# myshell-ai/OpenVoice

Hardware: AMD Instinct MI355X
Metric: real_time_factor (higher is better)
Workload: dtype f32; 1 GPU; ToneColorConverter.convert path, 32 x 10 s @ 22.05 kHz per GPU (T=861 frames), fp32, calibrated random weights; batch_per_gpu=32, global_batch=32, parallelism=dp1 (utterance sharding, RCCL broadcast of src/tgt se)

## Files before the change

include/openvoice_amd.h:

```cpp
#ifndef OPENVOICE_AMD_H
#define OPENVOICE_AMD_H

#include <stddef.h>
#include <stdint.h>

#ifdef __cplusplus
extern "C" {
#endif

typedef void* ov_stream_t;

enum {
  OV_OK = 0,
  OV_E_BADARG = -1,
  OV_E_UNSUPPORTED = -2,
  OV_E_ALIGN = -3,
  OV_E_LAUNCH = -4
};

enum {
  OV_EPI_LINEAR = 0,
  OV_EPI_GATE = 1,
  OV_EPI_RESSKIP = 2,
  OV_EPI_COUPLE = 3,
// ... 85 lines not shown
  const float* w_rs;
  const float* b_rs;
  const float* mask;
  int64_t bstride;
  int64_t cond_bstride;
  int64_t mask_bstride;
  int32_t B, H, T;
  int32_t ld;
  int32_t K;
  int32_t first;
  int32_t last;
  int32_t width;
  int32_t ntile;
  int32_t row_split;
  unsigned long long* dbg;
  float* acts;
} ov_wn_layer_params;
int ov_wn_layer_f32(const ov_wn_layer_params* p, ov_stream_t stream);
int ov_wn_layer_supported(int H, int K);
size_t ov_wn_pack_size(int rows, int cin, int K);
int ov_wn_pack_f32(const float* w, int rows, int cin, int K, float* dst);
int ov_wn_layer_tile(int B, int T, int width);

int ov_frame_hops_f32(const float* wave, float* hops, int B, int N, int hop, int pad, int U, int ld,
                      ov_stream_t stream);

int ov_frame_hops_windows_f32(const float* wave, int64_t n_samples, const int64_t* first_frame, int W, int hop, int pad,
                              int U, int ld, float* hops, ov_stream_t stream);
int ov_frame_hops_multi_f32(const float* pool, int64_t pool_len, const int64_t* records, int W, int hop, int pad, int U,
                            int ld, float* hops, ov_stream_t stream);
int ov_stitch_window_cores_f32(const float* o_hat, const int64_t* windows, int W, int Tw, int spf, float* out,
                               int64_t out_len, int64_t out_frame0, ov_stream_t stream);
int ov_carry_rows_f32(const int64_t* records, int n_records, const float* src_base, int64_t src_elems, float* dst_base,
                      int64_t dst_elems, ov_stream_t stream);
int ov_rows_f32_to_cl_bf16(const float* src, int64_t src_bs, int src_ld, uint16_t* dst, int B, int C, int L,
                           ov_stream_t stream);
int ov_cl_bf16_to_rows_f32(const uint16_t* src, float* dst, int64_t dst_bs, int dst_ld, int B, int C, int L,
                           ov_stream_t stream);

int ov_vad_frame_energy_f32(const float* pool, int64_t pool_len, const int64_t* records, int R, int H, int ldT,
                            float* energy, ov_stream_t stream);
int ov_vad_segments_i32(const float* energy, const int64_t* records, int R, int H, int ldT, float floor_lin,
                        float range_lin, int min_silence_frames, int min_speech_frames, int pad_frames, int32_t* mask,
                        int64_t* offsets, int64_t* n_active, ov_stream_t stream);
int ov_vad_compact_f32(const float* pool, int64_t pool_len, const int64_t* records, int R, int H, int ldT,
                       const int32_t* mask, const int64_t* offsets, const int64_t* out_bases, float* out,
// ... 189 lines not shown
```

openvoice_amd/_lib.py:

```python
import ctypes
import os

_HERE = os.path.dirname(os.path.abspath(__file__))
LIB_PATH = os.environ.get("OPENVOICE_AMD_LIB") or os.path.join(_HERE, "libopenvoice_amd.so")

OV_OK = 0
MIN_VERSION = 212
OV_ERRORS = {-1: "OV_E_BADARG", -2: "OV_E_UNSUPPORTED", -3: "OV_E_ALIGN", -4: "OV_E_LAUNCH"}

EPI_LINEAR, EPI_GATE, EPI_RESSKIP, EPI_COUPLE, EPI_POSTERIOR, EPI_CONVT, EPI_MAGNITUDE = range(7)
F_MASK_V = 1
F_OUT2_INIT = 2
F_CONVT_GROUPED = 4
F_NO_XCD_MAP = 8

_fp = ctypes.c_void_p
_i = ctypes.c_int
_i64 = ctypes.c_int64
LN_PRE_RELU, LN_POST_GELU = 1, 2


class ConvParams(ctypes.Structure):
    _fields_ = [
        ("x", _fp), ("w", _fp), ("bias", _fp), ("bias_b", _fp), ("out", _fp), ("res", _fp),
# ... 65 lines not shown
class WnLayerParams(ctypes.Structure):
    _fields_ = [("x", _fp), ("out", _fp), ("skip", _fp), ("w_in", _fp), ("b_in", _fp), ("cond", _fp), ("w_rs", _fp),
                ("b_rs", _fp), ("mask", _fp),
                ("bstride", ctypes.c_int64), ("cond_bstride", ctypes.c_int64), ("mask_bstride", ctypes.c_int64),
                ("B", ctypes.c_int32), ("H", ctypes.c_int32), ("T", ctypes.c_int32), ("ld", ctypes.c_int32),
                ("K", ctypes.c_int32), ("first", ctypes.c_int32), ("last", ctypes.c_int32), ("width", ctypes.c_int32),
                ("ntile", ctypes.c_int32), ("row_split", ctypes.c_int32), ("dbg", _fp), ("acts", _fp)]


SIGNATURES = {
    "ov_version": (ctypes.c_int, []),
    "ov_build_experiment": (ctypes.c_int, []),
    "ov_conv1d_pack_size": (ctypes.c_size_t, [ctypes.c_int, ctypes.c_int, ctypes.c_int]),
    "ov_conv1d_pack_rows": (ctypes.c_int, [ctypes.c_int]),
    "ov_conv1d_pack_f32": (ctypes.c_int, [_fp, ctypes.c_int, ctypes.c_int, ctypes.c_int, _fp]),
    "ov_conv1d_f32": (ctypes.c_int, [ctypes.POINTER(ConvParams), _fp]),
    "ov_resblock_pair_f32": (ctypes.c_int, [ctypes.POINTER(RespairParams), _fp]),
    "ov_resblock_pair_supported": (ctypes.c_int, [_i, _i, _i]),
    "ov_wn_layer_f32": (ctypes.c_int, [ctypes.POINTER(WnLayerParams), _fp]),
    "ov_wn_layer_supported": (ctypes.c_int, [_i, _i]),
    "ov_wn_pack_size": (ctypes.c_size_t, [_i, _i, _i]),
    "ov_wn_pack_f32": (ctypes.c_int, [_fp, _i, _i, _i, _fp]),
    "ov_wn_layer_tile": (ctypes.c_int, [_i, _i, _i]),
    "ov_conv_post_tanh_f32": (ctypes.c_int, [_fp, _fp, _fp, ctypes.c_int, ctypes.c_int, ctypes.c_int,
                                             ctypes.c_int, ctypes.c_float, _fp]),
    "ov_conv_post_tanh_limited_f32": (ctypes.c_int, [_fp, _fp, _fp, ctypes.c_int, ctypes.c_int, ctypes.c_int,
                                                     ctypes.c_int, ctypes.c_float, _fp, ctypes.c_int, _fp]),
    "ov_frame_limits_i32": (ctypes.c_int, [_fp, _fp, _i, _i, _i, _fp]),
    "ov_linear_f32": (ctypes.c_int, [_fp, _fp, _fp, _fp, ctypes.c_int, ctypes.c_int, ctypes.c_int, _fp]),
    "ov_sequence_mask_f32": (ctypes.c_int, [_fp, _fp, ctypes.c_int, ctypes.c_int, ctypes.c_int, _fp]),
    "ov_unpad_rows_f32": (ctypes.c_int, [_fp, _fp, ctypes.c_int, ctypes.c_int, ctypes.c_int, _fp]),
    "ov_polyphase_fir_f32": (ctypes.c_int, [_fp, _fp, _fp, ctypes.c_int64, ctypes.c_int64, _i, _i, _i, _fp]),
    "ov_polyphase_fir_rows_f32": (ctypes.c_int, [_fp, _i, _fp, _i64, _fp, _i64, _fp, _i64, _i64, _fp]),
    "ov_layernorm_freq_f32": (ctypes.c_int, [_fp, _fp, _fp, _fp, ctypes.c_int, ctypes.c_int, ctypes.c_int,
                                             ctypes.c_float, _fp]),
    "ov_conv2d_s2_relu_f32": (ctypes.c_int, [_fp, _fp, _fp, _fp, ctypes.c_int, ctypes.c_int, ctypes.c_int,
                                             ctypes.c_int, ctypes.c_int, _fp]),
    "ov_gru_f32": (ctypes.c_int, [_fp, _fp, _fp, _fp, ctypes.c_int, ctypes.c_int, ctypes.c_int, _fp]),
    "ov_conv1d_bf16_pack_size": (ctypes.c_size_t, [_i, _i, _i]),
    "ov_conv1d_bf16_pack": (ctypes.c_int, [_fp, _i, _i, _i, _fp]),
    "ov_conv1d_bf16_pack16": (ctypes.c_int, [_fp, _i, _i, _i, _fp]),
    "ov_conv1d_bf16cl": (ctypes.c_int, [ctypes.POINTER(ConvBf16Params), _fp]),
    "ov_resblock_pair_bf16cl": (ctypes.c_int, [ctypes.POINTER(RespairBf16Params), _fp]),
    "ov_resblock_pair_bf16_supported": (ctypes.c_int, [_i, _i, _i]),
    "ov_resblock_pair2_bf16cl": (ctypes.c_int, [ctypes.POINTER(Respair2Bf16Params), _fp]),
    "ov_resblock_pair2_bf16_supported": (ctypes.c_int, [_i, _i, _i]),
# ... 68 lines not shown
        _lib = lib
    return _lib


def torch_op(name, *args):
    try:
        return getattr(torch_ops(), name)(*args)
    except RuntimeError as exc:
        if isinstance(exc, OvError):
            raise
        raise OvError(str(exc).split("\n")[0]) from None


def check(code, what):
    if code != OV_OK:
        raise OvError(f"{what} failed: {OV_ERRORS.get(code, code)}")


SHIM_PATH = os.path.join(_HERE, "libopenvoice_amd_torch.so")
_ops = None
VALUE_FUNCS = {"ov_version", "ov_build_experiment", "ov_conv1d_pack_size", "ov_conv1d_pack_rows", "ov_wn_pack_size",
               "ov_conv1d_bf16_pack_size", "ov_resblock_pair_supported", "ov_wn_layer_supported", "ov_wn_layer_tile",
               "ov_resblock_pair_bf16_supported", "ov_resblock_pair2_bf16_supported", "ov_conv1d_split3_pack_size",
               "ov_conv1d_split3_supported", "ov_conv1d_wino_supported", "ov_conv1d_wino_chunk", "ov_conv1d_wino_pack_size"}


def binding():
    b = os.environ.get("OPENVOICE_AMD_BINDING", "ctypes" if os.environ.get("OPENVOICE_AMD_LIB") else "torch")
    if b not in ("torch", "ctypes"):
        raise OvError(f"OPENVOICE_AMD_BINDING={b!r}: expected 'torch' or 'ctypes'")
    return b


def use_torch_binding():
    return binding() == "torch"


def torch_ops():
    global _ops
    if _ops is None:
        import torch
        for path in (LIB_PATH, SHIM_PATH):
            if not os.path.exists(path):
                raise OvError(f"{path} not found: build the HIP extension first (python -c 'import __graft_entry__ "
                              f"as g; g.build()'); there is no CPU fallback (OPENVOICE_AMD_BINDING=ctypes needs only "
                              f"libopenvoice_amd.so)")
        torch.ops.load_library(SHIM_PATH)
# ... 49 lines not shown
```

openvoice_amd/csrc/torch_shim.cpp:

```cpp
#include <ATen/ATen.h>
#include <ATen/hip/impl/HIPGuardImplMasqueradingAsCUDA.h>
#include <c10/hip/HIPStream.h>
#include <torch/library.h>

#include <string>
#include <type_traits>

#include "openvoice_amd.h"

namespace {

const char* ov_strerror(int rc) {
  switch (rc) {
    case OV_E_BADARG: return "OV_E_BADARG";
    case OV_E_UNSUPPORTED: return "OV_E_UNSUPPORTED";
    case OV_E_ALIGN: return "OV_E_ALIGN";
    case OV_E_LAUNCH: return "OV_E_LAUNCH";
    default: return "unknown error";
  }
}

using OptTensor = c10::optional<at::Tensor>;

struct Ctx {
// ... 180 lines not shown
  DeviceScope scope(c);
  finish(ov_conv1d_f32(&p, c.stream()), "ov_conv1d_f32");
}

void resblock_pair_f32(const OptTensor& x, const OptTensor& w1, const OptTensor& b1, const OptTensor& w2,
                       const OptTensor& b2, const OptTensor& out, const OptTensor& add, const OptTensor& dbg,
                       const OptTensor& col_limit, at::IntArrayRef ip, at::ArrayRef<double> fp) {
  TORCH_CHECK(ip.size() == 11 && fp.size() == 2, "openvoice_amd::resblock_pair_f32: 11 integer and 2 float parameters");
  Ctx c{"resblock_pair_f32", false};
  ov_respair_params p{};
  p.x = sptr<float>(x, c, 0); p.w1 = sptr<float>(w1, c, 1); p.b1 = sptr<float>(b1, c, 2);
  p.w2 = sptr<float>(w2, c, 3); p.b2 = sptr<float>(b2, c, 4); p.out = sptr<float>(out, c, 5);
  p.add = sptr<float>(add, c, 6);
  p.dbg = sptr<unsigned long long>(dbg, c, 7);
  p.col_limit = sptr<int32_t>(col_limit, c, 8);
  p.B = (int32_t)ip[0]; p.C = (int32_t)ip[1]; p.L = (int32_t)ip[2]; p.ld = (int32_t)ip[3]; p.K = (int32_t)ip[4];
  p.dil = (int32_t)ip[5]; p.nwg = (int32_t)ip[6];
  p.x_bstride = ip[7]; p.out_bstride = ip[8]; p.add_bstride = ip[9]; p.col_limit_scale = (int32_t)ip[10];
  p.slope = (float)fp[0]; p.scale = (float)fp[1];
  DeviceScope scope(c);
  finish(ov_resblock_pair_f32(&p, c.stream()), "ov_resblock_pair_f32");
}

void wn_layer_f32(const OptTensor& x, const OptTensor& out, const OptTensor& skip, const OptTensor& w_in,
                  const OptTensor& b_in, const OptTensor& cond, const OptTensor& w_rs, const OptTensor& b_rs,
                  const OptTensor& mask, const OptTensor& dbg, const OptTensor& acts, at::IntArrayRef ip) {
  TORCH_CHECK(ip.size() == 13, "openvoice_amd::wn_layer_f32: 13 integer parameters");
  Ctx c{"wn_layer_f32", false};
  ov_wn_layer_params p{};
  p.x = sptr<float>(x, c, 0); p.out = sptr<float>(out, c, 1); p.skip = sptr<float>(skip, c, 2);
  p.w_in = sptr<float>(w_in, c, 3); p.b_in = sptr<float>(b_in, c, 4); p.cond = sptr<float>(cond, c, 5, ip[11]);
  p.w_rs = sptr<float>(w_rs, c, 6); p.b_rs = sptr<float>(b_rs, c, 7); p.mask = sptr<float>(mask, c, 8);
  p.dbg = sptr<unsigned long long>(dbg, c, 9);
  p.acts = sptr<float>(acts, c, 10);
  p.B = (int32_t)ip[0]; p.H = (int32_t)ip[1]; p.T = (int32_t)ip[2]; p.ld = (int32_t)ip[3]; p.K = (int32_t)ip[4];
  p.first = (int32_t)ip[5]; p.last = (int32_t)ip[6]; p.width = (int32_t)ip[7];
  p.bstride = ip[8]; p.cond_bstride = ip[9]; p.mask_bstride = ip[10]; p.row_split = (int32_t)ip[12];
  DeviceScope scope(c);
  finish(ov_wn_layer_f32(&p, c.stream()), "ov_wn_layer_f32");
}

void conv1d_bf16cl(const OptTensor& x, const OptTensor& w, const OptTensor& bias, const OptTensor& out,
                   const OptTensor& res, const OptTensor& add, const OptTensor& dbg, at::IntArrayRef ip,
                   at::ArrayRef<double> fp) {
  TORCH_CHECK(ip.size() == 9 && fp.size() == 3, "openvoice_amd::conv1d_bf16cl: 9 integer and 3 float parameters");
  Ctx c{"conv1d_bf16cl", false};
  ov_conv1d_bf16_params p{};
  p.x = sptr<uint16_t>(x, c, 0); p.w = sptr<uint16_t>(w, c, 1); p.bias = sptr<float>(bias, c, 2);
  p.out = sptr<uint16_t>(out, c, 3); p.res = sptr<uint16_t>(res, c, 4); p.add = sptr<uint16_t>(add, c, 5);
  p.dbg = sptr<unsigned long long>(dbg, c, 6);
  p.B = (int32_t)ip[0]; p.L = (int32_t)ip[1]; p.Cin = (int32_t)ip[2]; p.Cout = (int32_t)ip[3]; p.K = (int32_t)ip[4];
  p.dil = (int32_t)ip[5]; p.phase_s = (int32_t)ip[6]; p.bias_bstride = (int32_t)ip[7]; p.layout = (int32_t)ip[8];
  p.in_slope = (float)fp[0]; p.scale = (float)fp[1]; p.out_slope = (float)fp[2];
  DeviceScope scope(c);
  finish(ov_conv1d_bf16cl(&p, c.stream()), "ov_conv1d_bf16cl");
}

void resblock_pair_bf16cl(const OptTensor& x, const OptTensor& w1, const OptTensor& b1, const OptTensor& w2,
                          const OptTensor& b2, const OptTensor& out, const OptTensor& add, const OptTensor& dbg,
                          at::IntArrayRef ip, at::ArrayRef<double> fp) {
  TORCH_CHECK(ip.size() == 6 && fp.size() == 2, "openvoice_amd::resblock_pair_bf16cl: 6 integer and 2 float parameters");
  Ctx c{"resblock_pair_bf16cl", false};
// ... 50 lines not shown
  Ctx c{"conv1d_wino_f32", false};
  ov_conv1d_wino_params p{};
  p.x = sptr<float>(x, c, 0); p.w = sptr<float>(w, c, 1); p.bias = sptr<float>(bias, c, 2);
  p.out = sptr<float>(out, c, 3); p.res = sptr<float>(res, c, 4); p.add = sptr<float>(add, c, 5);
  p.dbg = sptr<unsigned long long>(dbg, c, 6);
  p.col_limit = sptr<int32_t>(col_limit, c, 7); p.col_limit_scale = (int32_t)ip[14];
  p.B = (int32_t)ip[0]; p.Cin = (int32_t)ip[1]; p.Cout = (int32_t)ip[2]; p.L = (int32_t)ip[3];
  p.x_ld = (int32_t)ip[4]; p.out_ld = (int32_t)ip[5]; p.K = (int32_t)ip[6]; p.dil = (int32_t)ip[7]; p.nwg = (int32_t)ip[8];
  p.x_bstride = ip[9]; p.out_bstride = ip[10]; p.res_bstride = ip[11]; p.add_bstride = ip[12]; p.frags = (int32_t)ip[13];
  p.in_slope = (float)fp[0]; p.scale = (float)fp[1]; p.out_slope = (float)fp[2];
  DeviceScope scope(c);
  finish(ov_conv1d_wino_f32(&p, c.stream()), "ov_conv1d_wino_f32");
}

}

TORCH_LIBRARY(openvoice_amd, m) {
  m.def("conv1d_f32(Tensor? x, Tensor? w, Tensor? bias, Tensor(a!)? out, Tensor? res, Tensor? add, Tensor(b!)? out2, "
        "Tensor? mask, Tensor? bias_b, Tensor? col_limit, int[] ip, float[] fp) -> ()", &conv1d_f32);
  m.def("resblock_pair_f32(Tensor? x, Tensor? w1, Tensor? b1, Tensor? w2, Tensor? b2, Tensor(a!)? out, Tensor? add, "
        "Tensor(b!)? dbg, Tensor? col_limit, int[] ip, float[] fp) -> ()", &resblock_pair_f32);
  m.def("wn_layer_f32(Tensor? x, Tensor(a!)? out, Tensor(b!)? skip, Tensor? w_in, Tensor? b_in, Tensor? cond, Tensor? w_rs, "
        "Tensor? b_rs, Tensor? mask, Tensor(c!)? dbg, Tensor(d!)? acts, int[] ip) -> ()", &wn_layer_f32);
  m.def("conv1d_bf16cl(Tensor? x, Tensor? w, Tensor? bias, Tensor(a!)? out, Tensor? res, Tensor? add, Tensor(b!)? dbg, "
        "int[] ip, float[] fp) -> ()", &conv1d_bf16cl);
  m.def("resblock_pair_bf16cl(Tensor? x, Tensor? w1, Tensor? b1, Tensor? w2, Tensor? b2, Tensor(a!)? out, Tensor? add, "
        "Tensor(b!)? dbg, int[] ip, float[] fp) -> ()", &resblock_pair_bf16cl);
  m.def("resblock_pair2_bf16cl(Tensor? x, Tensor? w1, Tensor? b1, Tensor? w2, Tensor? b2, Tensor(a!)? out, Tensor? add, "
        "Tensor(b!)? dbg, int[] ip, float[] fp) -> ()", &resblock_pair2_bf16cl);
  m.def("conv1d_split3(Tensor? x, Tensor? w, Tensor? bias, Tensor(a!)? out, Tensor? res, Tensor(b!)? dbg, "
        "Tensor? col_limit, int[] ip, float[] fp) -> ()", &conv1d_split3);
  m.def("conv1d_wino_f32(Tensor? x, Tensor? w, Tensor? bias, Tensor(a!)? out, Tensor? res, Tensor? add, Tensor(b!)? dbg, "
        "Tensor? col_limit, int[] ip, float[] fp) -> ()",
        &conv1d_wino_f32);
  bind_device<&ov_frame_hops_f32>(m, "frame_hops_f32");
  bind_device<&ov_frame_hops_windows_f32>(m, "frame_hops_windows_f32");
  bind_device<&ov_frame_hops_multi_f32>(m, "frame_hops_multi_f32");
  bind_device<&ov_carry_rows_f32>(m, "carry_rows_f32");
  bind_device<&ov_rows_f32_to_cl_bf16>(m, "rows_f32_to_cl_bf16");
  bind_device<&ov_cl_bf16_to_rows_f32>(m, "cl_bf16_to_rows_f32");
  bind_device<&ov_vad_frame_energy_f32>(m, "vad_frame_energy_f32");
  bind_device<&ov_vad_segments_i32>(m, "vad_segments_i32");
  bind_device<&ov_vad_compact_f32>(m, "vad_compact_f32");
  bind_device<&ov_stitch_window_cores_f32>(m, "stitch_window_cores_f32");
  bind_device<&ov_conv_post_tanh_f32>(m, "conv_post_tanh_f32");
  bind_device<&ov_conv_post_tanh_limited_f32>(m, "conv_post_tanh_limited_f32");
  bind_device<&ov_frame_limits_i32>(m, "frame_limits_i32");
  bind_device<&ov_linear_f32>(m, "linear_f32");
  bind_device<&ov_sequence_mask_f32>(m, "sequence_mask_f32");
  bind_device<&ov_unpad_rows_f32>(m, "unpad_rows_f32");
  bind_device<&ov_polyphase_fir_f32>(m, "polyphase_fir_f32");
  bind_device<&ov_polyphase_fir_rows_f32>(m, "polyphase_fir_rows_f32");
  bind_device<&ov_layernorm_freq_f32>(m, "layernorm_freq_f32");
  bind_device<&ov_conv2d_s2_relu_f32>(m, "conv2d_s2_relu_f32");
  bind_device<&ov_gru_f32>(m, "gru_f32");
  bind_device<&ov_embed_f32>(m, "embed_f32");
  bind_device<&ov_layernorm_ch_f32>(m, "layernorm_ch_f32");
  bind_device<&ov_rel_attention_f32>(m, "rel_attention_f32");
  bind_device<&ov_dwconv1d_f32>(m, "dwconv1d_f32");
  bind_device<&ov_expand1_f32>(m, "expand1_f32");
  bind_device<&ov_add_bias_mask_f32>(m, "add_bias_mask_f32");
  bind_device<&ov_rq_spline_inverse_f32>(m, "rq_spline_inverse_f32");
  bind_device<&ov_duration_f32>(m, "duration_f32");
  bind_device<&ov_expand_prior_f32>(m, "expand_prior_f32");
  bind_device<&ov_conv_post_tanh_bf16>(m, "conv_post_tanh_bf16");
  bind_device<&ov_split3_from_f32>(m, "split3_from_f32");
  bind_device<&ov_split3_to_f32>(m, "split3_to_f32");
  bind_host<&ov_conv1d_pack_f32>(m, "conv1d_pack_f32");
  bind_host<&ov_wn_pack_f32>(m, "wn_pack_f32");
  bind_host<&ov_conv1d_bf16_pack>(m, "conv1d_bf16_pack");
  bind_host<&ov_conv1d_bf16_pack16>(m, "conv1d_bf16_pack16");
  bind_host<&ov_conv1d_split3_pack>(m, "conv1d_split3_pack");
  bind_value<&ov_conv1d_split3_pack_size>(m, "conv1d_split3_pack_size");
  bind_value<&ov_conv1d_split3_supported>(m, "conv1d_split3_supported");
  bind_host<&ov_conv1d_wino_pack_f32>(m, "conv1d_wino_pack_f32");
  bind_value<&ov_conv1d_wino_pack_size>(m, "conv1d_wino_pack_size");
  bind_value<&ov_conv1d_wino_supported>(m, "conv1d_wino_supported");
  bind_value<&ov_conv1d_wino_chunk>(m, "conv1d_wino_chunk");
  bind_value<&ov_conv1d_pack_size>(m, "conv1d_pack_size");
  bind_value<&ov_conv1d_pack_rows>(m, "conv1d_pack_rows");
  bind_value<&ov_wn_pack_size>(m, "wn_pack_size");
  bind_value<&ov_conv1d_bf16_pack_size>(m, "conv1d_bf16_pack_size");
  bind_value<&ov_resblock_pair_supported>(m, "resblock_pair_supported");
  bind_value<&ov_wn_layer_supported>(m, "wn_layer_supported");
  bind_value<&ov_wn_layer_tile>(m, "wn_layer_tile");
  bind_value<&ov_resblock_pair_bf16_supported>(m, "resblock_pair_bf16_supported");
  bind_value<&ov_resblock_pair2_bf16_supported>(m, "resblock_pair2_bf16_supported");
  bind_value<&ov_version>(m, "version");
  bind_value<&ov_build_experiment>(m, "build_experiment");
}
```

openvoice_amd/engine.py:

```python
import ctypes
import os

import torch

from . import _lib
from ._lib import (ConvParams, EPI_CONVT, EPI_COUPLE, EPI_GATE, EPI_LINEAR, EPI_POSTERIOR, EPI_RESSKIP,
                   F_CONVT_GROUPED, F_MASK_V, F_OUT2_INIT)
from .params import ENC_Q_LAYERS, FLOW_LAYERS, N_FLOWS, REF_ENC_FILTERS, REF_ENC_GRU, effective_weight

GENERATOR_MARGIN = 16
LIMIT_MAX_BATCH = 256
LRELU_SLOPE = 0.1
FINAL_LRELU_SLOPE = 0.01


SUPPORTED_RESBLOCK_KERNELS = (3, 7, 11)
SUPPORTED_RESBLOCK_DILATIONS = (1, 3, 5)


def validate_config(cfg):
    def bad(field, value, why):
        raise _lib.OvError(f"config field {field!r} = {value!r} is not supported by the MI355X kernels: {why}")

    rb = str(cfg.get("resblock", "1"))
# ... 270 lines not shown
    return max(GENERATOR_MARGIN, generator_margin_frames(cfg), generator_margin_frames(cfg, chain_reach=chain_reach))


def wn_fused_row_order(hidden):
    assert hidden % 8 == 0
    idx = []
    for q in range(hidden // 8):
        for j in range(4):
            a, b = 8 * q + j, 8 * q + j + 4
            idx += [a, b, hidden + a, hidden + b]
    return torch.tensor(idx, dtype=torch.long)


def wn_pack(w_dense, device):
    w_dense = w_dense.detach().to(torch.float32).cpu().contiguous()
    rows, cin, k = w_dense.shape
    n = _lib.call("ov_wn_pack_size", rows, cin, k)
    assert n > 0, (rows, cin, k)
    packed = torch.empty(n, dtype=torch.float32)
    _lib.call("ov_wn_pack_f32", w_dense, rows, cin, k, packed)
    return packed.to(device)


def launch_wn_layer(layer, x, out, skip, mask, B, T, ld, cond=None, cond_off=0, cond_bs=0, first=False, last=False,
                    width=0, mask_bs=0, dbg=None, acts=None, row_split=0):
    if _lib.use_torch_binding():
        H = layer["hidden"]
        _lib.torch_op("wn_layer_f32", x, out, skip, layer["w_in"], layer["b_in"], cond, layer["w_rs"], layer["b_rs"],
                      mask, dbg, acts, [B, H, T, ld, layer["K"], int(first), int(last), width, H * ld, cond_bs, mask_bs,
                                        cond_off, row_split])
        return
    p = _lib.WnLayerParams()
    p.x, p.out, p.skip = _ptr(x), _ptr(out), _ptr(skip)
    p.w_in, p.b_in, p.w_rs, p.b_rs = _ptr(layer["w_in"]), _ptr(layer["b_in"]), _ptr(layer["w_rs"]), _ptr(layer["b_rs"])
    p.cond = _ptr(cond, cond_off) if cond is not None else None
    p.mask = _ptr(mask)
    H = layer["hidden"]
    p.bstride, p.cond_bstride, p.mask_bstride = H * ld, cond_bs, mask_bs
    p.B, p.H, p.T, p.ld, p.K = B, H, T, ld, layer["K"]
    p.first, p.last, p.width, p.row_split = int(first), int(last), width, row_split
    p.dbg = ctypes.c_void_p(dbg.data_ptr()) if dbg is not None else None
    p.acts = _ptr(acts) if acts is not None else None
    stream = ctypes.c_void_p(torch.cuda.current_stream(x.device).cuda_stream)
    _lib.check(_lib.load().ov_wn_layer_f32(ctypes.byref(p), stream), "ov_wn_layer_f32")


class _WaveNet:

    def __init__(self, sd, prefix, n_layers, hidden, device):
        order = gate_row_order(hidden)
        self.hidden, self.n_layers = hidden, n_layers
        self.in_layers, self.rs_layers, self.fused_layers = [], [], []
        K = sd[f"{prefix}.in_layers.0.weight_v"].shape[2] if f"{prefix}.in_layers.0.weight_v" in sd else \
            sd[f"{prefix}.in_layers.0.weight"].shape[2]
        self.fused = bool(_lib.call("ov_wn_layer_supported", hidden, K))
        forder = wn_fused_row_order(hidden) if self.fused else None
        for i in range(n_layers):
            w_in = effective_weight(sd, f"{prefix}.in_layers.{i}")
            b_in = sd[f"{prefix}.in_layers.{i}.bias"].float()
            self.in_layers.append(PackedConv(w_in[order], b_in[order], device, K=w_in.shape[2], cout=hidden))
            w_rs = effective_weight(sd, f"{prefix}.res_skip_layers.{i}")
            b_rs = sd[f"{prefix}.res_skip_layers.{i}.bias"].float()
            self.rs_layers.append(PackedConv(w_rs, b_rs, device, K=1))
            if self.fused:
                if w_rs.shape[0] == hidden:
                    w_rs = torch.cat([torch.zeros_like(w_rs), w_rs])
                    b_rs = torch.cat([torch.zeros_like(b_rs), b_rs])
                self.fused_layers.append(dict(hidden=hidden, K=w_in.shape[2], w_in=wn_pack(w_in[forder], device),
                                              b_in=b_in[forder].contiguous().to(device), w_rs=wn_pack(w_rs, device),
                                              b_rs=b_rs.contiguous().to(device)))
        wc = effective_weight(sd, prefix + ".cond_layer")[:, :, 0]
        bc = sd[prefix + ".cond_layer.bias"].float()
        full = torch.cat([order + 2 * hidden * i for i in range(n_layers)])
        self.cond_w = wc[full].contiguous().to(device)
        self.cond_b = bc[full].contiguous().to(device)
        if self.fused:
            full = torch.cat([forder + 2 * hidden * i for i in range(n_layers)])
            self.cond_w_fused = wc[full].contiguous().to(device)
            self.cond_b_fused = bc[full].contiguous().to(device)


class ConverterEngine:

    def __init__(self, state_dict, model_cfg, spec_channels, device, zero_g=False):
        self.device = torch.device(device)
        if self.device.type != "cuda":
            raise _lib.OvError("ConverterEngine needs a ROCm device ('cuda:N'); there is no CPU path")
        sd = {k: v.detach().float().cpu() for k, v in state_dict.items()}
        cfg = dict(model_cfg.items()) if hasattr(model_cfg, "items") else dict(model_cfg)
        validate_config(cfg)
        self.cfg = cfg
# ... 195 lines not shown
    def _zeros_like_cached(self, t):
        key = tuple(t.shape)
        z = self._zeros.get(key)
        if z is None:
            z = self._zeros[key] = torch.zeros_like(t)
        return z

    def _side_streams(self, n):
        while len(self._streams) < n:
            self._streams.append(torch.cuda.Stream(self.device))
        return self._streams[:n]

    def _chain_scratch(self, ws, n):
        extra = ws.setdefault("dec_extra", [])
        while len(extra) < n:
            extra.append(torch.empty_like(ws["dec"][0]))
        return extra

    def _wavenet(self, wn, ws, B, T, cond, mask):
        H, Tp = wn.hidden, ws["Tp"]
        cbs = 0 if cond.shape[0] == 1 else cond.shape[1]
        if self.fuse_wn and wn.fused:
            src, dst = ws["h"], ws["h2"]
            for i in range(wn.n_layers):
                layer = wn.fused_layers[i]
                args = dict(cond=cond, cond_off=2 * H * i, cond_bs=cbs, first=i == 0, last=i == wn.n_layers - 1,
                            mask_bs=Tp, acts=ws["acts"], row_split=self.wn_row_split)
                if self.profile is None:
                    launch_wn_layer(layer, src, dst, ws["skip"], mask, B, T, Tp, **args)
                else:
                    e0, e1 = torch.cuda.Event(enable_timing=True), torch.cuda.Event(enable_timing=True)
                    e0.record()
                    launch_wn_layer(layer, src, dst, ws["skip"], mask, B, T, Tp, **args)
                    e1.record()
                    rs_rows = H if args["last"] else 2 * H
                    self.profile.append(("wn_layer", 2.0 * (2 * H * H * layer["K"] + rs_rows * H) * T * B, e0, e1))
                src, dst = dst, src
            return
        for i in range(wn.n_layers):
            self._conv(wn.in_layers[i], ws["h"], 0, H * Tp, ws["acts"], 0, H * Tp, B, T, epi=EPI_GATE,
                       bias_b=cond, bias_b_off=2 * H * i, bias_b_bs=cbs, rows=2 * H, x_ld=Tp, out_ld=Tp, tag="wn_in")
            last = i == wn.n_layers - 1
            self._conv(wn.rs_layers[i], ws["acts"], 0, H * Tp, ws["h"], 0, H * Tp, B, T, epi=EPI_RESSKIP,
                       flags=F_OUT2_INIT if i == 0 else 0, out2=ws["skip"], out2_bs=H * Tp, mask=mask, mask_bs=Tp,
                       split=0 if last else H, x_ld=Tp, out_ld=Tp, tag="wn_rs")

    def _flow(self, src, buf, ws, B, T, conds, mask, reverse):
        C, half, H, Tp = self.inter, self.half, self.hidden, ws["Tp"]
        order = range(N_FLOWS - 1, -1, -1) if reverse else range(N_FLOWS)
        for n, f in enumerate(order):
# ... 516 lines not shown
```

Before: 3060 x real-time (audio s / wall s).

## Add Winograd-based fused WaveNet layer kernel for K=5, H=192

Adds a fused WaveNet layer kernel whose dilated K=5 input convolution uses a Winograd F(4,3)-style transform split into two 3-tap groups, running on MFMA f32 16x16x4 with double-buffered LDS transforms, then the gate and res/skip 1x1 conv in the same kernel. Weights are pre-transformed on the host into a new packed layout, and a policy based on tile count per occupancy round chooses it when enabled. The aim is to cut multiply count for the input conv. The trade-offs are extra transform arithmetic, reduced fp32 accuracy from the transform constants, and a fixed 128-wide tile that can hurt wave quantization.

```diff
diff --git a/include/openvoice_amd.h b/include/openvoice_amd.h
--- a/include/openvoice_amd.h
+++ b/include/openvoice_amd.h
@@ -131,6 +131,11 @@
 int ov_wn_pack_f32(const float* w, int rows, int cin, int K, float* dst);
 int ov_wn_layer_tile(int B, int T, int width);
 
+int ov_wn_layer_wino_f32(const ov_wn_layer_params* p, ov_stream_t stream);
+int ov_wn_layer_wino_tile(void);
+size_t ov_wn_wino_pack_size(int rows, int cin, int K);
+int ov_wn_wino_pack_f32(const float* w, int rows, int cin, int K, float* dst);
+
 int ov_frame_hops_f32(const float* wave, float* hops, int B, int N, int hop, int pad, int U, int ld,
                       ov_stream_t stream);
 
diff --git a/openvoice_amd/_lib.py b/openvoice_amd/_lib.py
--- a/openvoice_amd/_lib.py
+++ b/openvoice_amd/_lib.py
@@ -111,6 +111,10 @@
     "ov_wn_pack_size": (ctypes.c_size_t, [_i, _i, _i]),
     "ov_wn_pack_f32": (ctypes.c_int, [_fp, _i, _i, _i, _fp]),
     "ov_wn_layer_tile": (ctypes.c_int, [_i, _i, _i]),
+    "ov_wn_layer_wino_f32": (ctypes.c_int, [ctypes.POINTER(WnLayerParams), _fp]),
+    "ov_wn_layer_wino_tile": (ctypes.c_int, []),
+    "ov_wn_wino_pack_size": (ctypes.c_size_t, [_i, _i, _i]),
+    "ov_wn_wino_pack_f32": (ctypes.c_int, [_fp, _i, _i, _i, _fp]),
     "ov_conv_post_tanh_f32": (ctypes.c_int, [_fp, _fp, _fp, ctypes.c_int, ctypes.c_int, ctypes.c_int,
                                              ctypes.c_int, ctypes.c_float, _fp]),
     "ov_conv_post_tanh_limited_f32": (ctypes.c_int, [_fp, _fp, _fp, ctypes.c_int, ctypes.c_int, ctypes.c_int,
@@ -225,7 +229,8 @@
 VALUE_FUNCS = {"ov_version", "ov_build_experiment", "ov_conv1d_pack_size", "ov_conv1d_pack_rows", "ov_wn_pack_size",
                "ov_conv1d_bf16_pack_size", "ov_resblock_pair_supported", "ov_wn_layer_supported", "ov_wn_layer_tile",
                "ov_resblock_pair_bf16_supported", "ov_resblock_pair2_bf16_supported", "ov_conv1d_split3_pack_size",
-               "ov_conv1d_split3_supported", "ov_conv1d_wino_supported", "ov_conv1d_wino_chunk", "ov_conv1d_wino_pack_size"}
+               "ov_conv1d_split3_supported", "ov_conv1d_wino_supported", "ov_conv1d_wino_chunk", "ov_conv1d_wino_pack_size",
+               "ov_wn_layer_wino_tile", "ov_wn_wino_pack_size"}
 
 
 def binding():
diff --git a/openvoice_amd/csrc/torch_shim.cpp b/openvoice_amd/csrc/torch_shim.cpp
--- a/openvoice_amd/csrc/torch_shim.cpp
+++ b/openvoice_amd/csrc/torch_shim.cpp
@@ -226,11 +226,13 @@
   finish(ov_resblock_pair_f32(&p, c.stream()), "ov_resblock_pair_f32");
 }
 
-void wn_layer_f32(const OptTensor& x, const OptTensor& out, const OptTensor& skip, const OptTensor& w_in,
-                  const OptTensor& b_in, const OptTensor& cond, const OptTensor& w_rs, const OptTensor& b_rs,
-                  const OptTensor& mask, const OptTensor& dbg, const OptTensor& acts, at::IntArrayRef ip) {
-  TORCH_CHECK(ip.size() == 13, "openvoice_amd::wn_layer_f32: 13 integer parameters");
-  Ctx c{"wn_layer_f32", false};
+template <int (*FN)(const ov_wn_layer_params*, ov_stream_t)>
+void wn_layer_any(const char* op, const char* entry, const OptTensor& x, const OptTensor& out, const OptTensor& skip,
+                  const OptTensor& w_in, const OptTensor& b_in, const OptTensor& cond, const OptTensor& w_rs,
+                  const OptTensor& b_rs, const OptTensor& mask, const OptTensor& dbg, const OptTensor& acts,
+                  at::IntArrayRef ip) {
+  TORCH_CHECK(ip.size() == 13, "openvoice_amd::", op, ": 13 integer parameters");
+  Ctx c{op, false};
   ov_wn_layer_params p{};
   p.x = sptr<float>(x, c, 0); p.out = sptr<float>(out, c, 1); p.skip = sptr<float>(skip, c, 2);
   p.w_in = sptr<float>(w_in, c, 3); p.b_in = sptr<float>(b_in, c, 4); p.cond = sptr<float>(cond, c, 5, ip[11]);
@@ -241,7 +243,18 @@
   p.first = (int32_t)ip[5]; p.last = (int32_t)ip[6]; p.width = (int32_t)ip[7];
   p.bstride = ip[8]; p.cond_bstride = ip[9]; p.mask_bstride = ip[10]; p.row_split = (int32_t)ip[12];
   DeviceScope scope(c);
-  finish(ov_wn_layer_f32(&p, c.stream()), "ov_wn_layer_f32");
+  finish(FN(&p, c.stream()), entry);
+}
+void wn_layer_f32(const OptTensor& x, const OptTensor& out, const OptTensor& skip, const OptTensor& w_in,
+                  const OptTensor& b_in, const OptTensor& cond, const OptTensor& w_rs, const OptTensor& b_rs,
+                  const OptTensor& mask, const OptTensor& dbg, const OptTensor& acts, at::IntArrayRef ip) {
+  wn_layer_any<&ov_wn_layer_f32>("wn_layer_f32", "ov_wn_layer_f32", x, out, skip, w_in, b_in, cond, w_rs, b_rs, mask, dbg, acts, ip);
+}
+void wn_layer_wino_f32(const OptTensor& x, const OptTensor& out, const OptTensor& skip, const OptTensor& w_in,
+                       const OptTensor& b_in, const OptTensor& cond, const OptTensor& w_rs, const OptTensor& b_rs,
+                       const OptTensor& mask, const OptTensor& dbg, const OptTensor& acts, at::IntArrayRef ip) {
+  wn_layer_any<&ov_wn_layer_wino_f32>("wn_layer_wino_f32", "ov_wn_layer_wino_f32", x, out, skip, w_in, b_in, cond, w_rs, b_rs, mask, dbg,
+                                      acts, ip);
 }
 
 void conv1d_bf16cl(const OptTensor& x, const OptTensor& w, const OptTensor& bias, const OptTensor& out,
@@ -338,6 +351,8 @@
         "Tensor(b!)? dbg, Tensor? col_limit, int[] ip, float[] fp) -> ()", &resblock_pair_f32);
   m.def("wn_layer_f32(Tensor? x, Tensor(a!)? out, Tensor(b!)? skip, Tensor? w_in, Tensor? b_in, Tensor? cond, Tensor? w_rs, "
         "Tensor? b_rs, Tensor? mask, Tensor(c!)? dbg, Tensor(d!)? acts, int[] ip) -> ()", &wn_layer_f32);
+  m.def("wn_layer_wino_f32(Tensor? x, Tensor(a!)? out, Tensor(b!)? skip, Tensor? w_in, Tensor? b_in, Tensor? cond, Tensor? w_rs, "
+        "Tensor? b_rs, Tensor? mask, Tensor(c!)? dbg, Tensor(d!)? acts, int[] ip) -> ()", &wn_layer_wino_f32);
   m.def("conv1d_bf16cl(Tensor? x, Tensor? w, Tensor? bias, Tensor(a!)? out, Tensor? res, Tensor? add, Tensor(b!)? dbg, "
         "int[] ip, float[] fp) -> ()", &conv1d_bf16cl);
   m.def("resblock_pair_bf16cl(Tensor? x, Tensor? w1, Tensor? b1, Tensor? w2, Tensor? b2, Tensor(a!)? out, Tensor? add, "
@@ -384,6 +399,9 @@
   bind_device<&ov_split3_to_f32>(m, "split3_to_f32");
   bind_host<&ov_conv1d_pack_f32>(m, "conv1d_pack_f32");
   bind_host<&ov_wn_pack_f32>(m, "wn_pack_f32");
+  bind_host<&ov_wn_wino_pack_f32>(m, "wn_wino_pack_f32");
+  bind_value<&ov_wn_wino_pack_size>(m, "wn_wino_pack_size");
+  bind_value<&ov_wn_layer_wino_tile>(m, "wn_layer_wino_tile");
   bind_host<&ov_conv1d_bf16_pack>(m, "conv1d_bf16_pack");
   bind_host<&ov_conv1d_bf16_pack16>(m, "conv1d_bf16_pack16");
   bind_host<&ov_conv1d_split3_pack>(m, "conv1d_split3_pack");
diff --git a/openvoice_amd/csrc/wn_layer_wino.hip b/openvoice_amd/csrc/wn_layer_wino.hip
--- /dev/null
+++ b/openvoice_amd/csrc/wn_layer_wino.hip
@@ -0,0 +1,354 @@
+#include <hip/hip_runtime.h>
+
+#include "conv1d_wino.h"
+#include "openvoice_amd.h"
+
+namespace ovkwn {
+
+using ovk::f32x2;
+using ovk::f32x4;
+using ovkw::lds_barrier;
+using ovkw::wino_products;
+using ovkw::wino_zero_product;
+
+constexpr int K = 5, H = 192;
+static_assert(ovkw::wino_lead(K) == 0 && ovkw::wino_trail(K) == 1 && wino_products(K) == 11, "(w0 w1 w2)(w3 w4 0)");
+constexpr int NWAVE = 8;
+constexpr int RB = 2 * H / (16 * NWAVE);
+constexpr int NF = 2;
+constexpr int NT = 16 * NF;
+constexpr int W = 4 * NT;
+constexpr int NB = W / 16;
+constexpr int CI = 16;
+constexpr int NCH = H / CI;
+constexpr int NSLOT = wino_products(K);
+constexpr int SLOT = CI * NT;
+constexpr int VBUF = NSLOT * SLOT;
+constexpr int NU = H / 4;
+constexpr int XS = 144;
+constexpr int NR2 = H / 16;
+static_assert(NWAVE * 64 == CI * NT, "one (channel, tile) per lane and chunk");
+
+__device__ __forceinline__ float gate(float t, float s) {
+  const float a = __builtin_amdgcn_exp2f(fabsf(t) * -2.8853900817779268f);
+  const float e = __builtin_amdgcn_exp2f(s * -1.4426950408889634f);
+  const float r = __builtin_amdgcn_rcpf((1.f + a) * (1.f + e));
+  return copysignf((1.f - a) * r, t);
+}
+
+__global__ __launch_bounds__(64 * NWAVE, 2) void wn_layer_wino_kernel(const ov_wn_layer_params p) {
+  __shared__ __attribute__((aligned(16))) float Vs[2 * VBUF];
+  __shared__ __attribute__((aligned(16))) float acts[H * XS];
+  __shared__ __attribute__((aligned(16))) float msk[W];
+
+  const int tid = threadIdx.x;
+  const int lane = tid & 63;
+  const int wave = __builtin_amdgcn_readfirstlane(tid >> 6);
+  const int T = p.T;
+  const uint32_t ld = (uint32_t)p.ld;
+  const int b = (int)blockIdx.x / p.ntile;
+  const int t0 = ((int)blockIdx.x - b * p.ntile) * W;
+  const int g = lane >> 4, c = lane & 15;
+  const int64_t boff = (int64_t)b * p.bstride;
+
+  if (tid < W / 4) {
+    const int t = t0 + 4 * tid;
+    f32x4 m = {0.f, 0.f, 0.f, 0.f};
+    if (t < T) m = *reinterpret_cast<const f32x4*>(p.mask + (int64_t)b * p.mask_bstride + t);
+#pragma unroll
+    for (int r = 0; r < 4; ++r) m[r] = t + r < T ? m[r] : 0.f;
+    *reinterpret_cast<f32x4*>(msk + 4 * tid) = m;
+  }
+
+  const int tt = tid & (NT - 1), cil = tid / NT;
+  const int tc = t0 + 4 * tt;
+  const float* __restrict__ xrow = p.x + boff + (size_t)cil * ld;
+  uint32_t okm = 0;
+#pragma unroll
+  for (int m = 0; m < 8; ++m) okm |= (tc - 2 + m >= 0 && tc - 2 + m < T ? 1u : 0u) << m;
+  const uint32_t offa = (okm & 1u) ? (uint32_t)(tc - 2) : 0u;
+  const uint32_t offb = (okm & 4u) ? (uint32_t)tc : 0u;
+  const uint32_t offc = (okm & 64u) ? (uint32_t)(tc + 4) : 0u;
+  f32x2 sa, sc;
+  f32x4 sb;
+  auto request = [&](int chunk) {
+    const float* r = xrow + (size_t)(chunk * CI) * ld;
+    sa = *reinterpret_cast<const f32x2*>(r + offa);
+    sb = *reinterpret_cast<const f32x4*>(r + offb);
+    sc = *reinterpret_cast<const f32x2*>(r + offc);
+  };
+  const int vdst = cil * NT + (tt ^ ((cil & 1) << 4));
+  auto transform = [&](int buf) {
+    float* v = Vs + buf * VBUF + vdst;
+    float d[9];
+    d[0] = sa[0]; d[1] = sa[1]; d[2] = sb[0]; d[3] = sb[1]; d[4] = sb[2]; d[5] = sb[3]; d[6] = sc[0]; d[7] = sc[1];
+#pragma unroll
+    for (int m = 0; m < 8; ++m) d[m] = ((okm >> m) & 1u) ? d[m] : 0.f;
+    d[8] = 0.f;
+    ovkw::static_for<0, 2>([&](auto gc) {
+      constexpr int gg = decltype(gc)::value;
+      const float d0 = d[3 * gg], d1 = d[3 * gg + 1], d2 = d[3 * gg + 2], d3 = d[3 * gg + 3], d4 = d[3 * gg + 4],
+                  d5 = d[3 * gg + 5];
+      const float t1 = __builtin_fmaf(-4.f, d2, d4), t2 = __builtin_fmaf(-4.f, d1, d3), t3 = d4 - d2, t4 = d3 - d1;
+      v[(6 * gg + 0) * SLOT] = __builtin_fmaf(4.f, d0, __builtin_fmaf(-5.f, d2, d4));
+      v[(6 * gg + 1) * SLOT] = t1 + t2;
+      v[(6 * gg + 2) * SLOT] = t1 - t2;
+      v[(6 * gg + 3) * SLOT] = __builtin_fmaf(2.f, t4, t3);
+      v[(6 * gg + 4) * SLOT] = __builtin_fmaf(-2.f, t4, t3);
+      if constexpr (!wino_zero_product(K, gg, 5)) v[(6 * gg + 5) * SLOT] = __builtin_fmaf(4.f, d1, __builtin_fmaf(-5.f, d3, d5));
+    });
+  };
+
+  const int frag0 = wave * RB, row0 = 16 * frag0;
+  f32x4 acc[RB][NF][6];
+  {
+    const float* __restrict__ cb = p.cond ? p.cond + (int64_t)b * p.cond_bstride : nullptr;
+#pragma unroll
+    for (int i = 0; i < RB; ++i) {
+      f32x4 bv = *reinterpret_cast<const f32x4*>(p.b_in + row0 + 16 * i + 4 * g);
+      if (cb) bv += *reinterpret_cast<const f32x4*>(cb + row0 + 16 * i + 4 * g);
+#pragma unroll
+      for (int f = 0; f < NF; ++f)
+#pragma unroll
+        for (int q = 0; q < 6; ++q) acc[i][f][q] = q == 1 ? bv : f32x4{0.f, 0.f, 0.f, 0.f};
+    }
+  }
+  const f32x4* __restrict__ w1 = reinterpret_cast<const f32x4*>(p.w_in) + (size_t)wave * (NU * RB * 3 * 64) + lane;
+  f32x4 a_cur[RB][3];
+#pragma unroll
+  for (int i = 0; i < RB; ++i)
+#pragma unroll
+    for (int j = 0; j < 3; ++j) a_cur[i][j] = w1[(i * 3 + j) * 64];
+  int voff[NF];
+#pragma unroll
+  for (int f = 0; f < NF; ++f) voff[f] = g * NT + 16 * (f ^ (g & 1)) + c;
+
+  request(0);
+  transform(0);
+  request(1);
+  lds_barrier();
+#pragma unroll 1
+  for (int chunk = 0; chunk < NCH; ++chunk) {
+    if (chunk + 1 < NCH) transform((chunk + 1) & 1);
+    if (chunk + 2 < NCH) request(chunk + 2);
+    const float* vb = Vs + (chunk & 1) * VBUF;
+    float bq[NF][NSLOT];
+#pragma unroll
+    for (int f = 0; f < NF; ++f)
+#pragma unroll
+      for (int s = 0; s < NSLOT; ++s) bq[f][s] = vb[s * SLOT + voff[f]];
+    const f32x4* __restrict__ wn = w1 + (size_t)(chunk * (CI / 4) + 1) * (RB * 3 * 64);
+#pragma unroll
+    for (int ul = 0; ul < CI / 4; ++ul) {
+#pragma unroll
+      for (int i = 0; i < RB; ++i) {
+        __builtin_amdgcn_sched_barrier(0);
+#pragma unroll
+        for (int s = 0; s < NSLOT; ++s) {
+#pragma unroll
+          for (int f = 0; f < NF; ++f)
+            acc[i][f][s % 6] = __builtin_amdgcn_mfma_f32_16x16x4f32(a_cur[i][s >> 2][s & 3], bq[f][s], acc[i][f][s % 6], 0, 0, 0);
+          if (i == RB - 1 && ul + 1 < CI / 4) {
+#pragma unroll
+            for (int f = 0; f < NF; ++f) bq[f][s] = vb[s * SLOT + (ul + 1) * 4 * NT + voff[f]];
+          }
+        }
+        __builtin_amdgcn_sched_barrier(0);
+#pragma unroll
+        for (int j = 0; j < 3; ++j) a_cur[i][j] = wn[(size_t)ul * (RB * 3 * 64) + (i * 3 + j) * 64];
+      }
+    }
+    lds_barrier();
+  }
+
+#pragma unroll
+  for (int i = 0; i < RB; ++i) {
+    const int ch = 8 * (frag0 + i) + g;
+#pragma unroll
+    for (int f = 0; f < NF; ++f) {
+      f32x4 o[4];
+#pragma unroll
+      for (int r = 0; r < 4; ++r) {
+        const float y0 = acc[i][f][0][r], y1 = acc[i][f][1][r], y2 = acc[i][f][2][r], y3 = acc[i][f][3][r],
+                    y4 = acc[i][f][4][r], y5 = acc[i][f][5][r];
+        const float s1 = y1 + y2, e1 = y1 - y2, s2 = y3 + y4, e2 = y3 - y4;
+        o[r][0] = (y0 + s1) + s2;
+        o[r][1] = __builtin_fmaf(2.f, e2, e1);
+        o[r][2] = __builtin_fmaf(4.f, s2, s1);
+        o[r][3] = __builtin_fmaf(8.f, e2, e1) + y5;
+      }
+      f32x4 ga, gb;
+#pragma unroll
+      for (int e = 0; e < 4; ++e) {
+        ga[e] = gate(o[0][e], o[2][e]);
+        gb[e] = gate(o[1][e], o[3][e]);
+      }
+      *reinterpret_cast<f32x4*>(acts + ch * XS + 64 * f + 4 * c) = ga;
+      *reinterpret_cast<f32x4*>(acts + (ch + 4) * XS + 64 * f + 4 * c) = gb;
+    }
+  }
+
+  const f32x4* __restrict__ w2 = reinterpret_cast<const f32x4*>(p.w_rs) + (size_t)wave * ((NR2 + 1) * RB * 64);
+  const bool skip_rows = row0 >= H;
+  const bool idle2 = p.last && !skip_rows;
+  f32x4 a2[RB], a2n[RB];
+  f32x4 acc2[RB][NB];
+  if (!idle2) {
+#pragma unroll
+    for (int i = 0; i < RB; ++i) a2[i] = w2[i * 64 + lane];
+    const float* __restrict__ src =
+        (skip_rows ? p.skip + boff + (size_t)(row0 - H) * ld : p.x + boff + (size_t)row0 * ld) + (size_t)c * ld;
+    const bool zero_src = skip_rows && p.first;
+#pragma unroll
+    for (int i = 0; i < RB; ++i)
+#pragma unroll
+      for (int j = 0; j < NB; ++j) {
+        const int col = t0 + 16 * j + 4 * g;
+        const uint32_t voff2 = (uint32_t)(16 * i) * ld + (uint32_t)(col < T ? col : 0);
+        if (zero_src) acc2[i][j] = f32x4{0.f, 0.f, 0.f, 0.f};
+        else acc2[i][j] = *reinterpret_cast<const f32x4*>(src + voff2);
+      }
+  }
+  __syncthreads();
+  if (idle2) return;
+#pragma unroll
+  for (int i = 0; i < RB; ++i) {
+    const float bv = p.b_rs[row0 + 16 * i + c];
+#pragma unroll
+    for (int j = 0; j < NB; ++j) acc2[i][j] += bv;
+  }
+  {
+    const float* al = acts + g * XS + c;
+    float bcur[NB], bnxt[NB];
+#pragma unroll
+    for (int j = 0; j < NB; ++j) bcur[j] = al[16 * j];
+#pragma unroll 1
+    for (int grp = 0; grp < NR2 / 4; ++grp) {
+      const float* ag = al + grp * 64 * XS;
+      const f32x4* __restrict__ wg = w2 + (size_t)grp * (4 * RB * 64);
+#pragma unroll
+      for (int m = 0; m < 16; ++m) {
+        const int u = m & 3;
+        if (u == 0) {
+#pragma unroll
+          for (int i = 0; i < RB; ++i) a2n[i] = (wg + (size_t)(m / 4 + 1) * (RB * 64))[i * 64 + lane];
+        }
+        {
+          const int s = (m + 1) % 16;
+          const float* an = (m + 1 < 16) ? ag : (grp + 1 < NR2 / 4 ? ag + 64 * XS : ag);
+#pragma unroll
+          for (int j = 0; j < NB; ++j) bnxt[j] = an[4 * s * XS + 16 * j];
+        }
+        __builtin_amdgcn_sched_barrier(0);
+#pragma unroll
+        for (int i = 0; i < RB; ++i)
+#pragma unroll
+          for (int j = 0; j < NB; ++j)
+            acc2[i][j] = __builtin_amdgcn_mfma_f32_16x16x4f32(bcur[j], a2[i][u], acc2[i][j], 0, 0, 0);
+        __builtin_amdgcn_sched_barrier(0);
+#pragma unroll
+        for (int j = 0; j < NB; ++j) bcur[j] = bnxt[j];
+        if (u == 3) {
+#pragma unroll
+          for (int i = 0; i < RB; ++i) a2[i] = a2n[i];
+        }
+      }
+    }
+  }
+
+  float* __restrict__ dst =
+      (skip_rows ? p.skip + boff + (size_t)(row0 - H) * ld : p.out + boff + (size_t)row0 * ld) + (size_t)c * ld;
+  if (t0 + W <= T) {
+#pragma unroll
+    for (int j = 0; j < NB; ++j) {
+      f32x4 mk = {1.f, 1.f, 1.f, 1.f};
+      if (!skip_rows) mk = *reinterpret_cast<const f32x4*>(msk + 16 * j + 4 * g);
+#pragma unroll
+      for (int i = 0; i < RB; ++i)
+        *reinterpret_cast<f32x4*>(dst + (uint32_t)(16 * i) * ld + (uint32_t)(t0 + 16 * j + 4 * g)) = acc2[i][j] * mk;
+    }
+  } else {
+#pragma unroll
+    for (int j = 0; j < NB; ++j) {
+      const int col = t0 + 16 * j + 4 * g;
+      if (col >= T) continue;
+      f32x4 mk = {1.f, 1.f, 1.f, 1.f};
+      if (!skip_rows) mk = *reinterpret_cast<const f32x4*>(msk + 16 * j + 4 * g);
+#pragma unroll
+      for (int i = 0; i < RB; ++i) {
+        const f32x4 v = acc2[i][j] * mk;
+        float* o = dst + (uint32_t)(16 * i) * ld + (uint32_t)col;
+#pragma unroll
+        for (int r = 0; r < 4; ++r)
+          if (col + r < T) o[r] = v[r];
+      }
+    }
+  }
+}
+
+}
+
+using namespace ovkwn;
+
+#if !defined(__HIP_DEVICE_COMPILE__)
+extern "C" {
+
+int ov_wn_layer_wino_tile(void) { return W; }
+
+size_t ov_wn_wino_pack_size(int rows, int cin, int Kw) {
+  if (rows != 2 * H || cin != H || Kw != K) return 0;
+  return ((size_t)NWAVE * NU + 1) * RB * 3 * 64 * 4;
+}
+
+int ov_wn_wino_pack_f32(const float* w, int rows, int cin, int Kw, float* dst) {
+  const size_t n = ov_wn_wino_pack_size(rows, cin, Kw);
+  if (!w || !dst || n == 0) return OV_E_BADARG;
+  static const double Gm[6][3] = {{1.0 / 4, 0, 0},           {-1.0 / 6, -1.0 / 6, -1.0 / 6}, {-1.0 / 6, 1.0 / 6, -1.0 / 6},
+                                  {1.0 / 24, 1.0 / 12, 1.0 / 6}, {1.0 / 24, -1.0 / 12, 1.0 / 6}, {0, 0, 1}};
+  for (size_t i = 0; i < n; ++i) dst[i] = 0.f;
+  for (int wv = 0; wv < NWAVE; ++wv)
+    for (int u = 0; u < NU; ++u)
+      for (int i = 0; i < RB; ++i)
+        for (int l = 0; l < 64; ++l)
+          for (int s = 0; s < NSLOT; ++s) {
+            const int grp = s / 6, pt = s % 6;
+            const int row = (wv * RB + i) * 16 + (l & 15), ci = 4 * u + (l >> 4);
+            double v = 0;
+            for (int k = 0; k < 3; ++k) {
+              const int tap = 3 * grp + k - ovkw::wino_lead(K);
+              if (tap >= 0 && tap < K) v += Gm[pt][k] * (double)w[((size_t)row * cin + ci) * K + tap];
+            }
+            dst[(((((size_t)wv * NU + u) * RB + i) * 3 + s / 4) * 64 + l) * 4 + s % 4] = (float)v;
+          }
+  return OV_OK;
+}
+
+int ov_wn_layer_wino_f32(const ov_wn_layer_params* pin, ov_stream_t stream) {
+  if (!pin || !pin->x || !pin->out || !pin->skip || !pin->w_in || !pin->b_in || !pin->w_rs || !pin->b_rs || !pin->mask)
+    return OV_E_BADARG;
+  ov_wn_layer_params q = *pin;
+  if (q.B <= 0 || q.T <= 0 || q.H <= 0 || q.K <= 0) return OV_E_BADARG;
+  if (q.H != H || q.K != K) return OV_E_UNSUPPORTED;
+  if (q.ld == 0) q.ld = q.T;
+  if (q.ld < q.T || q.out == q.x || q.dbg) return OV_E_BADARG;
+  if (q.mask_bstride == 0) q.mask_bstride = q.ld;
+  if ((int64_t)q.H * q.ld > UINT32_MAX / 2) return OV_E_BADARG;
+  if ((q.ld % 4) || (q.bstride % 4) || (q.cond_bstride % 4) || (reinterpret_cast<uintptr_t>(q.x) & 15) ||
+      (reinterpret_cast<uintptr_t>(q.w_in) & 15) || (reinterpret_cast<uintptr_t>(q.w_rs) & 15) ||
+      (reinterpret_cast<uintptr_t>(q.b_in) & 15) || (reinterpret_cast<uintptr_t>(q.b_rs) & 15) ||
+      (q.cond && (reinterpret_cast<uintptr_t>(q.cond) & 15)) || (reinterpret_cast<uintptr_t>(q.out) & 15) ||
+      (reinterpret_cast<uintptr_t>(q.skip) & 15))
+    return OV_E_ALIGN;
+  if ((reinterpret_cast<uintptr_t>(q.mask) & 15) || (q.mask_bstride % 4)) return OV_E_ALIGN;
+  if (q.mask_bstride < (int64_t)((q.T + 3) / 4) * 4) return OV_E_BADARG;
+  if (q.width != 0 && q.width != W) return OV_E_BADARG;
+  q.width = W;
+  q.ntile = (q.T + W - 1) / W;
+  if ((int64_t)q.B * q.ntile > INT32_MAX) return OV_E_BADARG;
+  hipLaunchKernelGGL(wn_layer_wino_kernel, dim3((unsigned)(q.B * q.ntile)), dim3(64 * NWAVE), 0,
+                     static_cast<hipStream_t>(stream), q);
+  return hipGetLastError() == hipSuccess ? OV_OK : OV_E_LAUNCH;
+}
+
+}
+#endif
diff --git a/openvoice_amd/engine.py b/openvoice_amd/engine.py
--- a/openvoice_amd/engine.py
+++ b/openvoice_amd/engine.py
@@ -316,17 +316,42 @@
     return packed.to(device)
 
 
+WN_WINO_MIN_ITEMS = 168
+WN_WINO_ROUND = 256
+
+
+def wn_wino_items(B, T):
+    return B * ((T + 127) // 128)
+
+
+def wn_wino_policy(B, T):
+    items = wn_wino_items(B, T)
+    rounds = (items + WN_WINO_ROUND - 1) // WN_WINO_ROUND
+    return items >= WN_WINO_MIN_ITEMS * rounds
+
+
+def wn_wino_pack(w_dense, device):
+    w_dense = w_dense.detach().to(torch.float32).cpu().contiguous()
+    rows, cin, k = w_dense.shape
+    n = _lib.call("ov_wn_wino_pack_size", rows, cin, k)
+    assert n > 0, (rows, cin, k)
+    packed = torch.empty(n, dtype=torch.float32)
+    _lib.call("ov_wn_wino_pack_f32", w_dense, rows, cin, k, packed)
+    return packed.to(device)
+
+
 def launch_wn_layer(layer, x, out, skip, mask, B, T, ld, cond=None, cond_off=0, cond_bs=0, first=False, last=False,
-                    width=0, mask_bs=0, dbg=None, acts=None, row_split=0):
+                    width=0, mask_bs=0, dbg=None, acts=None, row_split=0, winograd=False):
+    entry, w_in = ("wn_layer_wino_f32", layer["w_in_wino"]) if winograd else ("wn_layer_f32", layer["w_in"])
     if _lib.use_torch_binding():
         H = layer["hidden"]
-        _lib.torch_op("wn_layer_f32", x, out, skip, layer["w_in"], layer["b_in"], cond, layer["w_rs"], layer["b_rs"],
+        _lib.torch_op(entry, x, out, skip, w_in, layer["b_in"], cond, layer["w_rs"], layer["b_rs"],
                       mask, dbg, acts, [B, H, T, ld, layer["K"], int(first), int(last), width, H * ld, cond_bs, mask_bs,
                                         cond_off, row_split])
         return
     p = _lib.WnLayerParams()
     p.x, p.out, p.skip = _ptr(x), _ptr(out), _ptr(skip)
-    p.w_in, p.b_in, p.w_rs, p.b_rs = _ptr(layer["w_in"]), _ptr(layer["b_in"]), _ptr(layer["w_rs"]), _ptr(layer["b_rs"])
+    p.w_in, p.b_in, p.w_rs, p.b_rs = _ptr(w_in), _ptr(layer["b_in"]), _ptr(layer["w_rs"]), _ptr(layer["b_rs"])
     p.cond = _ptr(cond, cond_off) if cond is not None else None
     p.mask = _ptr(mask)
     H = layer["hidden"]
@@ -336,7 +361,7 @@
     p.dbg = ctypes.c_void_p(dbg.data_ptr()) if dbg is not None else None
     p.acts = _ptr(acts) if acts is not None else None
     stream = ctypes.c_void_p(torch.cuda.current_stream(x.device).cuda_stream)
-    _lib.check(_lib.load().ov_wn_layer_f32(ctypes.byref(p), stream), "ov_wn_layer_f32")
+    _lib.check(getattr(_lib.load(), "ov_" + entry)(ctypes.byref(p), stream), "ov_" + entry)
 
 
 class _WaveNet:
@@ -361,6 +386,7 @@
                     w_rs = torch.cat([torch.zeros_like(w_rs), w_rs])
                     b_rs = torch.cat([torch.zeros_like(b_rs), b_rs])
                 self.fused_layers.append(dict(hidden=hidden, K=w_in.shape[2], w_in=wn_pack(w_in[forder], device),
+                                              w_in_wino=wn_wino_pack(w_in[forder], device),
                                               b_in=b_in[forder].contiguous().to(device), w_rs=wn_pack(w_rs, device),
                                               b_rs=b_rs.contiguous().to(device)))
         wc = effective_weight(sd, prefix + ".cond_layer")[:, :, 0]
@@ -602,10 +628,11 @@
         cbs = 0 if cond.shape[0] == 1 else cond.shape[1]
         if self.fuse_wn and wn.fused:
             src, dst = ws["h"], ws["h2"]
+            winograd = self.use_winograd and wn_wino_policy(B, T)
             for i in range(wn.n_layers):
                 layer = wn.fused_layers[i]
                 args = dict(cond=cond, cond_off=2 * H * i, cond_bs=cbs, first=i == 0, last=i == wn.n_layers - 1,
-                            mask_bs=Tp, acts=ws["acts"], row_split=self.wn_row_split)
+                            mask_bs=Tp, acts=ws["acts"], row_split=self.wn_row_split, winograd=winograd)
                 if self.profile is None:
                     launch_wn_layer(layer, src, dst, ws["skip"], mask, B, T, Tp, **args)
                 else:
```

Result: faster. 3100 x real-time (audio s / wall s) (median of 6 runs) (+1.3%).
